# Qw11111111111/SequenceAligning

Hardware: AMD Instinct MI355X
Metric: GCUPS (affine-gap NW) at 1/2/4/8 MI355X; % of HBM roofline (higher is better)
Workload: dtype i32-exact (i16x2 packed arithmetic)

## Files before the change

sequencealigning_amd/csrc/nw_kernels.hip:

```cpp
#include <hip/hip_runtime.h>

#include <algorithm>
#include <type_traits>
#include <utility>

#include "nw_common.hpp"
#include "nw_host.hpp"
#include "saln_options.hpp"
#include "saln.h"

namespace saln {

template <int G>
__device__ __forceinline__ int32_t shr1(int32_t old, int32_t v) {
    static_assert(G == 16 || G == 64, "group must be a DPP row or the wave");
    if constexpr (G == 16)
        return __builtin_amdgcn_update_dpp(old, v, 0x111 , 0xf, 0xf, false);
    else
        return __builtin_amdgcn_update_dpp(old, v, 0x138 , 0xf, 0xf, false);
}

__device__ __forceinline__ uint32_t pack_block(uint32_t bpp, uint32_t i = blockIdx.x) {
    const uint32_t sup = 8u * bpp;
    const uint32_t r = i % sup;
// ... 893 lines not shown
            push(SALN_CIGAR_D, n);
            i -= (int32_t)n;
        }
        st = __builtin_amdgcn_readlane(nxt, L);
    }
    if (NWV > 1) {
        if (lane == 0) req[0] = -1;
        __syncthreads();
    }
    if (run_len) {
        if (lane == 0 && out) out[nops] = (run_len << 4) | run_op;
        ++nops;
    }
    if constexpr (kSpec) {
        if (lane == 0) {
            const int32_t cur = sa.pass & 1;
            rec->in_i = ei;
            rec->in_j = ej;
            rec->in_k = ek;
            rec->out_i[cur] = xi;
            rec->out_j[cur] = xj;
            rec->out_k[cur] = ev < 0 ? xk : kSpecEv + ev;
            rec->nops = nops;
            rec->am_end = am_end;
        }
        return;
    }
    if (ev != kEvOrigin) nops = 0;
    if (out && nops > 1) {
        __builtin_amdgcn_s_waitcnt(0x0F70);
        __builtin_amdgcn_fence(__ATOMIC_SEQ_CST, "workgroup");
        for (uint32_t a = (uint32_t)lane; a < nops / 2; a += 64) {
            const uint32_t x = out[a], y = out[nops - 1 - a];
            out[a] = y;
            out[nops - 1 - a] = x;
        }
    }
    if (lane == 0) {
        saln_nw_result r = make_result(hend, WalkOut{ev, nops}, am_end);
        results[p.pair_id] = r;
    }
}

__global__ __launch_bounds__(256) void nw_spec_link_kernel(
    const NwPairDesc *__restrict__ pairs, SpecArgs sa, uint32_t *__restrict__ done,
    const int32_t *__restrict__ end_h, saln_nw_result *__restrict__ results,
    uint32_t *__restrict__ strict_err) {
    __shared__ uint32_t s_n[kSpecMaxStripes], s_first[kSpecMaxStripes], s_last[kSpecMaxStripes];
    __shared__ uint8_t s_k0[kSpecMaxStripes];
    __shared__ uint32_t s_part[256];
    __shared__ int32_t t_sh, bad_sh;
    const SpecPair sp = sa.pairs[blockIdx.x];
    const int32_t S = (int32_t)sp.n_stripes, P = sa.pass & 1;
    SpecStripe *rec = sa.stripes + sp.stripe_base;
    const uint32_t *ops = sa.ops + (uint64_t)sp.stripe_base * kSpecOpsCap;
    const int32_t tid = (int32_t)threadIdx.x;
    if (tid == 0) {
        t_sh = -1;
        bad_sh = 0;
    }
    __syncthreads();
    for (int32_t s = tid; s < S; s += 256)
        if (rec[s].out_k[P] >= kSpecEv) atomicMax(&t_sh, s);
    __syncthreads();
    const int32_t t = t_sh;
    const int32_t tk = t >= 0 ? rec[t].out_k[P] : kSpecNone;
    bool bad = t < 0 || tk == kSpecNone || tk == kSpecEv + kEvDead;
    for (int32_t s = max(t, 0) + tid; !bad && s < S - 1; s += 256) {
        const SpecStripe &a = rec[s], &b = rec[s + 1];
        if (a.in_i != b.out_i[P] || a.in_j != b.out_j[P] || a.in_k != b.out_k[P]) bad_sh = 1;
    }
    __syncthreads();
    const uint32_t idx = sp.plan_idx;
    if (bad || bad_sh) {
        if (tid == 0) {
            done[idx] = 0u;
            if (strict_err) atomicOr(strict_err, 2u);
        }
        return;
    }
    for (int32_t s = tid; s < S; s += 256) {
        const uint32_t n = s >= t ? rec[s].nops : 0u;
        s_n[s] = n;
        s_first[s] = n ? ops[(uint64_t)s * kSpecOpsCap] : 0u;
        s_last[s] = n ? ops[(uint64_t)s * kSpecOpsCap + n - 1] : 0u;
        if (s < t) rec[s].k0 = (int32_t)n;
    }
    __syncthreads();
    for (int32_t s = tid; s < S; s += 256)
        s_k0[s] = (s >= t && s < S - 1 && s_n[s] && (s_first[s] & 15u) == (s_last[s + 1] & 15u))
                      ? 1u : 0u;
    __syncthreads();
    const int32_t C = (S + 255) / 256;
    const int32_t u0 = tid * C, u1 = min(S, u0 + C);
    uint32_t part = 0;
    for (int32_t u = u0; u < u1; ++u) part += s_n[S - 1 - u] - s_k0[S - 1 - u];
    s_part[tid] = part;
    __syncthreads();
    for (int32_t d = 1; d < 256; d <<= 1) {
        const uint32_t v = tid >= d ? s_part[tid - d] : 0u;
        __syncthreads();
        s_part[tid] += v;
        __syncthreads();
    }
    uint32_t g = s_part[tid] - part;
    for (int32_t u = u0; u < u1; ++u) {
        const int32_t s = S - 1 - u;
        const uint32_t n = s_n[s], k0 = s_k0[s];
        rec[s].base = (int32_t)g - (int32_t)k0;
        rec[s].k0 = (int32_t)k0;
        if (n > k0) {
            uint32_t len = s_last[s] >> 4;
            for (int32_t r = s - 1; r >= t && s_k0[r]; --r) {
                len += s_first[r] >> 4;
                if (s_n[r] != 1u) break;
            }
            rec[s].open_w = (len << 4) | (s_last[s] & 15u);
        }
        g += n - k0;
    }
    if (tid == 255) {
        const uint32_t N = s_part[255];
        const NwPairDesc p = pairs[idx];
        const int ev = tk - kSpecEv;
        results[p.pair_id] = make_result(end_h[idx], WalkOut{ev, ev == kEvOrigin ? N : 0u},
                                         rec[S - 1].am_end);
        done[idx] = 1u;
    }
}

__global__ __launch_bounds__(64) void nw_spec_copy_kernel(
    const NwPairDesc *__restrict__ pairs, SpecArgs sa, const saln_nw_result *__restrict__ results,
    uint32_t *__restrict__ cigar) {
    const uint2 b = sa.blocks[blockIdx.x];
    const SpecPair sp = sa.pairs[b.x];
    if (!sa.done[sp.plan_idx]) return;
    const NwPairDesc p = pairs[sp.plan_idx];
    const int32_t N = (int32_t)results[p.pair_id].cigar_len;
    const SpecStripe &r = sa.stripes[sp.stripe_base + b.y];
    const int32_t n = (int32_t)r.nops;
    if (N == 0 || r.k0 >= n) return;
    const uint32_t *w = sa.ops + (uint64_t)(sp.stripe_base + b.y) * kSpecOpsCap;
    uint32_t *out = cigar + p.cigar_off;
    for (int32_t k = r.k0 + (int32_t)threadIdx.x; k < n; k += 64)
        out[N - 1 - (r.base + k)] = k == n - 1 ? r.open_w : w[k];
}

template <int K>
struct MaskWords {
    uint32_t w[(K + 3) / 4];
};


constexpr uint32_t kPub = 32;
constexpr uint32_t kColEmpty = 0x80000000u;

typedef short s16x2 __attribute__((ext_vector_type(2)));
typedef unsigned short u16x2 __attribute__((ext_vector_type(2)));

__device__ __forceinline__ s16x2 as_s2(uint32_t x) { return __builtin_bit_cast(s16x2, x); }
__device__ __forceinline__ uint32_t as_u(s16x2 x) { return __builtin_bit_cast(uint32_t, x); }
__device__ __forceinline__ s16x2 spl(int32_t v) { return s16x2{(short)v, (short)v}; }
__device__ __forceinline__ uint32_t pk2(int32_t lo, int32_t hi) {
    return ((uint32_t)lo & 0xFFFFu) | ((uint32_t)hi << 16);
}
__device__ __forceinline__ s16x2 vmax(s16x2 a, s16x2 b) { return __builtin_elementwise_max(a, b); }
__device__ __forceinline__ uint32_t pkb(int32_t lo, int32_t hi) {
    return ((uint32_t)(lo + 32768) & 0xFFFFu) | ((uint32_t)(hi + 32768) << 16);
}
__device__ __forceinline__ uint32_t umax2(uint32_t a, uint32_t b) {
    return __builtin_bit_cast(uint32_t, __builtin_elementwise_max(__builtin_bit_cast(u16x2, a),
                                                                  __builtin_bit_cast(u16x2, b)));
}
__device__ __forceinline__ uint32_t umin2(uint32_t a, uint32_t b) {
    return __builtin_bit_cast(uint32_t, __builtin_elementwise_min(__builtin_bit_cast(u16x2, a),
                                                                  __builtin_bit_cast(u16x2, b)));
}
__device__ __forceinline__ uint32_t cst2(int32_t c) { return (uint32_t)c * 0x10001u; }

template <int G>
__device__ __forceinline__ uint32_t gshift(uint32_t bnd, uint32_t v, bool group_start) {
    uint32_t s;
    if constexpr (G <= 16)
        s = __builtin_amdgcn_update_dpp(bnd, v, 0x111 , 0xf, 0xf, false);
    else
        s = __builtin_amdgcn_update_dpp(bnd, v, 0x138 , 0xf, 0xf, false);
    if constexpr (G == 16 || G == 64) return s;
    return group_start ? bnd : s;
}

__device__ __forceinline__ uint32_t col_pair_signs(uint32_t hi, uint32_t lo) {
    return __builtin_amdgcn_perm(hi, lo, 0x0B0A0908u);
}

__device__ __forceinline__ uint32_t bfi(uint32_t m, uint32_t a, uint32_t b) {
    return __builtin_amdgcn_bitop3_b32(m, a, b, 0xCA);
}

template <bool kArgMBit>
__device__ __forceinline__ uint32_t merge_walk(const uint32_t (&p)[8]) {
    uint32_t r = kArgMBit ? bfi(0x01010101u, p[0], p[1]) : p[1];
    r = bfi(0x03030303u, r, p[2]);
    r = bfi(0x07070707u, r, p[4]);
    r = bfi(0x1F1F1F1Fu, r, p[6]);
    return bfi(0x7F7F7F7Fu, r, p[7]);
}
__device__ __forceinline__ uint32_t merge_full(const uint32_t (&p)[8]) {
    uint32_t r = bfi(0x01010101u, p[0], p[1]);
    r = bfi(0x03030303u, r, p[2]);
    r = bfi(0x07070707u, r, p[3]);
    r = bfi(0x0F0F0F0Fu, r, p[4]);
    r = bfi(0x1F1F1F1Fu, r, p[5]);
    r = bfi(0x3F3F3F3Fu, r, p[6]);
    return bfi(0x7F7F7F7Fu, r, p[7]);
}

template <int K>
struct PkMask {
    uint32_t w[(K + 3) / 4];
};
template <int K>
__device__ __forceinline__ uint32_t pick_col(const uint32_t (&h)[K], int k) {
    uint32_t v[K];
#pragma unroll
    for (int i = 0; i < K; ++i) v[i] = h[i];
    int n = K;
#pragma unroll
    for (int bit = 0; (1 << bit) < K; ++bit) {
        const bool b = (k >> bit) & 1;
#pragma unroll
        for (int i = 0; 2 * i < n; ++i) v[i] = 2 * i + 1 < n ? (b ? v[2 * i + 1] : v[2 * i]) : v[2 * i];
        n = (n + 1) / 2;
    }
    return v[0];
}
template <int K>
struct NibSeg {
    uint32_t w[(K + 3) / 4 / 2 + 1];
};

struct PlanSrc {
    const NwPairDesc *pairs;
    uint32_t first;
    int32_t *end_h;
    __device__ __forceinline__ NwPairDesc pair(uint32_t i) const { return pairs[first + i]; }
    __device__ __forceinline__ void end(uint32_t i, const NwPairDesc &, int32_t h) const {
        end_h[first + i] = h;
    }
};

struct AvsaSrc {
    const uint64_t *q_off, *d_off;
    const uint32_t *q_ids, *d_ids;
    uint32_t nq;
    uint32_t nq_total;
    uint64_t base;
    int2 *out;
    __device__ __forceinline__ NwPairDesc pair(uint32_t i) const {
        const uint64_t k = base + i;
        const uint32_t qi = q_ids[k % nq], di = d_ids[k / nq];
        NwPairDesc p{};
        p.q_off = q_off[qi];
        p.db_off = d_off[di];
        p.len_q = (uint32_t)(q_off[qi + 1] - p.q_off);
        p.len_db = (uint32_t)(d_off[di + 1] - p.db_off);
        p.mask_off = (uint64_t)di * nq_total + qi;
        return p;
    }
    __device__ __forceinline__ void end(uint32_t, const NwPairDesc &p, int32_t h) const {
        out[p.mask_off] = make_int2(h >> 1, (h & 1) ? SALN_REF_PANIC_BOUNDARY : SALN_OK);
    }
};

struct AvsaSrcP : AvsaSrc {
    __device__ __forceinline__ NwPairDesc pair(uint32_t i) const {
        const uint64_t k = base + i, j = k >> 1;
        const uint32_t qi = q_ids[j % nq], di = d_ids[2 * (j / nq) + (k & 1)];
        NwPairDesc p{};
        p.q_off = q_off[qi];
        p.db_off = d_off[di];
        p.len_q = (uint32_t)(q_off[qi + 1] - p.q_off);
        p.len_db = (uint32_t)(d_off[di + 1] - p.db_off);
        p.mask_off = (uint64_t)di * nq_total + qi;
        return p;
    }
};


template <int G, int K, int kCodes>
constexpr int pk_min_waves() { return kCodes == 3  && G == 8 ? 3 : 1; }
typedef _Float16 f16x2 __attribute__((ext_vector_type(2)));
__device__ __forceinline__ uint32_t hmax3(uint32_t a, uint32_t b, uint32_t c) {
    return __builtin_bit_cast(
        uint32_t, __builtin_elementwise_maximum(__builtin_bit_cast(f16x2, a),
                                                __builtin_elementwise_maximum(
                                                    __builtin_bit_cast(f16x2, b),
                                                    __builtin_bit_cast(f16x2, c))));
}

struct RowIn {
    uint32_t w;
};

template <int G, int K, int kCodes, typename Src, int KS, bool kRebase = false, bool kProf = false,
          int kTabMode = 0>
__device__ __forceinline__ int fill_pk_body(Src src, uint32_t count, const uint8_t *__restrict__ qs,
                                            const uint8_t *__restrict__ ds,
                                            uint8_t *__restrict__ mask, Scoring sc,
                                            uint32_t ld_max, bool sc_steady,
                                            uint32_t vblock = ~0u) {
    constexpr bool kTab = kTabMode == 1 || kTabMode == 4 || kTabMode == 5;
    constexpr bool kRowProf = kTabMode == 5;
    constexpr bool kFree = kTab || kTabMode == 3;
    constexpr bool kS4 = kTabMode == 4;
    constexpr int kSc = kS4 ? 4 : 2;
    auto up = [](int32_t v2) -> int32_t { return kS4 ? (v2 >> 1) * 4 + (v2 & 1) : v2; };
    static_assert(kTabMode != 3 || kProf, "kTabMode 3: query profiles");
    constexpr int32_t kBias = kFree ? kFreeBias : 32768;
    auto pkx = [](int32_t lo, int32_t hi) {
        return ((uint32_t)(lo + kBias) & 0xFFFFu) | ((uint32_t)(hi + kBias) << 16);
    };
    static_assert(!kProf || (kCodes == kCodesNone && !kRebase), "profiles: score-only, one frame");
    static_assert(!kTab || ((kCodes == kCodesNib || kCodes == kCodesNone || kCodes == kCodesFull) &&
                            !kRebase && !kProf && !(kS4 && kCodes == kCodesFull)),
                  "tables: 4-bit codes, full codes (scale 2) or score-only, one frame");
    constexpr int GPB = 256 / G;
    constexpr Geom geo{G, K};
    extern __shared__ uint32_t drow[];
    const int lane = threadIdx.x % G;
    const uint32_t gi = pack_block(blocks_per_pack(2 * GPB), vblock == ~0u ? blockIdx.x : vblock) * GPB +
                        threadIdx.x / G;
    const uint32_t ia = 2 * gi, ib = 2 * gi + 1;
    if (ia >= count) return 0;
    const bool hasB = ib < count;
    const NwPairDesc pa = src.pair(ia);
    NwPairDesc pb = pa;
    if (hasB) pb = src.pair(ib);
    const int ldA = (int)pa.len_db, ldB = hasB ? (int)pb.len_db : 0;
    const int lqA = (int)pa.len_q, lqB = hasB ? (int)pb.len_q : 0;
    const uint8_t *__restrict__ qA = qs + pa.q_off;
    const uint8_t *__restrict__ qB = qs + pb.q_off;
    const uint8_t *__restrict__ dA = ds + pa.db_off;
    const uint8_t *__restrict__ dB = ds + pb.db_off;
    const int ldM = ldA > ldB ? ldA : ldB;
    const int32_t beta = -kSc * sc.gap_extend;
    const int32_t alpha = kFree ? beta : -2 * sc.match - beta;
    const uint32_t kPen = cst2(2 * (sc.match - sc.mismatch));
    const uint32_t kOpen = cst2(kSc * sc.gap_open);
    const uint32_t kDstep = cst2(2 * sc.gap_extend + alpha);
    const int32_t drift = kFree ? 0 : 2 * sc.gap_extend + alpha;
    const uint32_t cm = (uint32_t)(kSc * sc.match + alpha + beta) & 0xFFu;
    const uint32_t cmm = (uint32_t)(kSc * sc.mismatch + alpha + beta) & 0xFFu;
    const uint32_t kBonus = cm | cmm * 0x01010100u;
    const uint32_t kProfBase = cmm * 0x01010101u, kProfStep = cm - cmm;
    const uint32_t kCmm2 = cmm * 0x00010001u;
    constexpr uint32_t kAcgt = 'A' | 'C' << 8 | 'T' << 16 | 'G' << 24;
    auto acgt = [](uint32_t c) { return c == 'A' || c == 'C' || c == 'G' || c == 'T'; };
    bool bad = false;
    const uint32_t kRebaseAdd = cst2(-drift * kRebaseSteps);
    const int32_t ctr = kRebase ? rebase_center(sc, G * K) : 0;
    const bool gstart = lane == 0;

    const int col0 = lane * K;
    uint32_t qc[K], Hp[K], Dn[K];
    const uint32_t pen1 = 2 * (sc.match - sc.mismatch);
#pragma unroll
    for (int k = 0; k < K; ++k) {
        const int j = col0 + k + 1;
        if constexpr (kProf && kFree) {
            const uint32_t qch = j <= lqA ? (uint32_t)qA[j - 1] : 0u;
            qc[k] = (qch == 'A' ? cm : cmm) | (qch == 'C' ? cm : cmm) << 8 |
                    (qch == 'T' ? cm : cmm) << 16 | (qch == 'G' ? cm : cmm) << 24;
        } else if constexpr (kProf) {
            const uint32_t qch = j <= lqA ? (uint32_t)qA[j - 1] : 0u;
            qc[k] = (qch == 'A' ? 0u : pen1) | (qch == 'C' ? 0u : pen1 << 8) |
                    (qch == 'T' ? 0u : pen1 << 16) | (qch == 'G' ? 0u : pen1 << 24);
        } else if constexpr (kTab) {
            const uint32_t ca = j <= lqA ? (uint32_t)qA[j - 1] : 'A';
            const uint32_t cb = j <= lqB ? (uint32_t)qB[j - 1] : 'A';
            bad |= !acgt(ca) || !acgt(cb);
            qc[k] = kRowProf ? (((ca >> 1) & 3u) | 0x0C00u | (((cb >> 1) & 3u) + 4u) << 16 | 0x0C000000u)
                             : (((ca >> 1) & 3u) | ((cb >> 1) & 3u) << 16);
        } else {
            const uint32_t ca = j <= lqA ? (uint32_t)qA[j - 1] << 5 : 0xE000u;
            const uint32_t cb = j <= lqB ? (uint32_t)qB[j - 1] << 5 : 0xE000u;
            if constexpr (kTabMode == 2) bad |= (j <= lqA && !acgt(ca >> 5)) || (j <= lqB && !acgt(cb >> 5));
            qc[k] = ca | (cb << 16);
        }
        const int32_t h0 = up(hs_row0(sc, (uint32_t)j)) + beta * j - ctr;
        const int32_t d1 = up(ds_row1(sc, (uint32_t)j)) + alpha + beta * j - ctr;
        Hp[k] = pkx(h0, h0);
        Dn[k] = pkx(d1, d1);
    }
    uint32_t hd = pkx(up(hs_row0(sc, (uint32_t)col0)) + beta * col0 - ctr,
                      up(hs_row0(sc, (uint32_t)col0)) + beta * col0 - ctr);
    uint32_t pubF = 0, pubH = 0;
    uint32_t *__restrict__ myrow = drow + (threadIdx.x / G) * (ld_max + 2 * G) + G;
    uint16_t *__restrict__ myrow16 = reinterpret_cast<uint16_t *>(drow) +
                                     (threadIdx.x / G) * (ld_max + 2 * G) + G;
    for (int i = lane; i < ldM; i += G) {
        const uint32_t ca = i < ldA ? (uint32_t)dA[i] : 0u;
        const uint32_t cb = i < ldB ? (uint32_t)dB[i] : 0u;
        if constexpr (kRebase) {
            if constexpr (kTabMode == 2) bad |= (i < ldA && !acgt(ca)) || (i < ldB && !acgt(cb));
            myrow16[i] = (uint16_t)(ca | (cb << 8));
        } else if constexpr (kRowProf) {
            bad |= (i < ldA && !acgt(ca)) || (i < ldB && !acgt(cb));
            myrow[i] = ((ca >> 1) & 3u) << 3 | ((cb >> 1) & 3u) << 19 | 0x60006000u;
        } else if constexpr (kTab) {
            bad |= (i < ldA && !acgt(ca)) || (i < ldB && !acgt(cb));
            myrow[i] = ((ca >> 1) & 3u) | ((cb >> 1) & 3u) << 16 | 0x0C000C00u;
        } else {
            if constexpr (kTabMode == 2) bad |= (i < ldA && !acgt(ca)) || (i < ldB && !acgt(cb));
            myrow[i] = (ca << 5) | (cb << 21);
        }
    }
    asm volatile("s_waitcnt lgkmcnt(0)" : : : "memory");
    __builtin_amdgcn_wave_barrier();
    if constexpr (kTab) {
        if (__builtin_amdgcn_ballot_w64(bad)) return 1;
    } else if constexpr (kTabMode == 2) {
        if (!__builtin_amdgcn_ballot_w64(bad)) return 2;
    }
    const int lA = (lqA - 1) / K, kA = (lqA - 1) % K;
    const int lB = hasB ? (lqB - 1) / K : -1, kB = hasB ? (lqB - 1) % K : 0;
    const int tEA = lane == lA ? ldA + lane - 1 : -1;
    const int tEB = lane == lB ? ldB + lane - 1 : -1;
    static_assert(K % KS == 0 && (KS % 2 == 0 || KS == K), "segments hold whole column pairs");
    constexpr int NS = K / KS;
    uint8_t *__restrict__ mA = mask + pa.mask_off + (uint64_t)(lane * NS) * pa.mask_bs -
                               (int64_t)lane * (int64_t)pa.mask_rs;
    uint8_t *__restrict__ mB = mask + pb.mask_off + (uint64_t)(lane * NS) * pb.mask_bs -
                               (int64_t)lane * (int64_t)pb.mask_rs;
    const uint32_t *__restrict__ rowp = myrow - lane;
    const uint16_t *__restrict__ rowp16 = myrow16 - lane;
    const int T = (int)geo.steps((uint32_t)ldM);
    constexpr bool kWalkCodes = kCodes == kCodesWalk || kCodes == kCodesNib;
    static_assert(kCodes != kCodesNib || KS == K, "4-bit codes: one segment per lane");
    const int ldAs = (kWalkCodes && col0 >= lqA) ? 0 : ldA;
    const int ldBs = (kWalkCodes && col0 >= lqB) ? 0 : ldB;
    uint32_t HpB[K];

    uint32_t sF = 0, sH = 0;
    const uint32_t kRowAdd = cst2(drift);
    auto step = [&](int t, uint32_t(&Hin)[K], uint32_t(&Hout)[K], auto steady_c, RowIn row_in)
                    __attribute__((always_inline)) {
        constexpr bool kSteady = decltype(steady_c)::value;
        constexpr bool kRun = kSteady && !kRebase;
        const int r = t - lane + 1;
        uint32_t dch;
        if constexpr (kRun)
            dch = row_in.w;
        else if constexpr (kRebase)
            dch = __builtin_amdgcn_perm(0u, (uint32_t)rowp16[t], 0x0C010C00u) << 5;
        else
            dch = rowp[t];
        uint32_t prof_lo = 0, prof_hi = 0;
        if constexpr (kRowProf) {
            prof_lo = (kProfStep << (dch & 31u)) + kProfBase;
            prof_hi = (kProfStep << ((dch >> 16) & 31u)) + kProfBase;
        }
        int32_t base = 0;
        if constexpr (kRebase) {
            base = drift * (t & -kRebaseSteps) + ctr;
            if ((t & (kRebaseSteps - 1)) == 0 && t > 0) {
#pragma unroll
                for (int k = 0; k < K; ++k) {
                    Hin[k] += kRebaseAdd;
                    Dn[k] += kRebaseAdd;
                }
                hd += kRebaseAdd;
                pubF += kRebaseAdd;
                pubH += kRebaseAdd;
            }
        }
        const int32_t rb = t + 1;
        uint32_t gF, gH;
        if constexpr (kRun) {
            gF = sF;
            gH = sH;
            sF += kRowAdd;
            sH += kRowAdd;
        } else {
            const int32_t bF = up(is_col1(sc, (uint32_t)rb)) + alpha * rb + beta - base;
            const int32_t bH = up(hs_col0(sc, (uint32_t)rb)) + alpha * rb - base;
            gF = pkx(bF, bF);
            gH = pkx(bH, bH);
        }
        const uint32_t inF = gshift<G>(gF, pubF, gstart);
        const uint32_t inH = gshift<G>(gH, pubH, gstart);
        if (kSteady || (r >= 1 && r <= ldM)) {
            uint32_t F = inF;
            PkMask<KS> wa[NS], wb[NS];
            uint32_t cw[(K + 1) / 2];
            uint32_t prv[8];
            uint32_t nw[(K + 3) / 4], nlo = 0, nprv[4];
            const uint32_t endsel = (t == tEA ? 0x0000FFFFu : 0u) | (t == tEB ? 0xFFFF0000u : 0u);
            const uint32_t psel = kProf ? (((dch >> 6) & 0x00030003u) | 0x0C000C00u) : 0u;
            auto columns = [&](auto with_argm) __attribute__((always_inline)) {
            constexpr bool kM = decltype(with_argm)::value;
            uint32_t diag = hd;
#pragma unroll
            for (int k = 0; k < K; ++k) {
                const uint32_t hdk = diag;
                diag = Hin[k];
                const uint32_t pen = kProf     ? __builtin_amdgcn_perm(0u, qc[k], psel)
                                     : kRowProf ? __builtin_amdgcn_perm(prof_hi, prof_lo, qc[k])
                                     : kTab     ? __builtin_amdgcn_perm(0u, kBonus, qc[k] ^ dch)
                                                : umin2(qc[k] ^ dch, kPen);
                const uint32_t M = kFree ? hdk + pen : hdk - pen;
                const uint32_t I = F, D = Dn[k];
                const uint32_t H = kFree ? hmax3(M, I, D) : umax2(M, umax2(I, D));
                const uint32_t tO = M + kOpen;
                if constexpr (kCodes == kCodesNib) {
                    uint32_t s4[4];
                    if constexpr (kS4) {
                        const uint32_t Hm = H - 0x00020002u;
                        const uint32_t tO2 = M + (kOpen + 0x00020002u);
                        s4[0] = Hm - I;
                        s4[1] = Hm - D;
                        s4[2] = tO2 - I;
                        s4[3] = tO2 - D;
                        if constexpr (kM) s4[3] = bfi(endsel, M - Hm, s4[3]);
                    } else {
                    const uint32_t Hc = H & 0xFFFEFFFEu;
                    const uint32_t tOr = tO | 0x00010001u;
                    auto psub = [](uint32_t a, uint32_t b) { return as_u(as_s2(a) - as_s2(b)); };
                    s4[0] = psub(I, Hc);
                    s4[1] = psub(D, Hc);
                    s4[2] = psub(tOr, I);
                    s4[3] = psub(tOr, D);
                    if constexpr (kM) s4[3] = bfi(endsel, psub(M, Hc), s4[3]);
                    }
                    if (k % 2 == 0 && k < K - 1) {
#pragma unroll
                        for (int u = 0; u < 4; ++u) nprv[u] = s4[u];
                    } else {
                        uint32_t pw[4];
#pragma unroll
                        for (int u = 0; u < 4; ++u)
                            pw[u] = k % 2 ? col_pair_signs(s4[u], nprv[u])
                                          : col_pair_signs(kS4 && u < 2 ? 0x80008000u : 0u, s4[u]);
                        const int cp = k / 2, g = cp / 2;
                        auto bfi01 = [](uint32_t m, uint32_t a, uint32_t b) {
                            return kS4 ? __builtin_amdgcn_bitop3_b32(m, a, b, 0x35) : bfi(m, a, b);
                        };
                        if (cp % 2 == 0) {
                            uint32_t lo = bfi01(0x01010101u, pw[0], pw[1]);
                            lo = bfi(0x03030303u, lo, pw[2]);
                            lo = bfi(0x07070707u, lo, pw[3]);
                            if (cp == (K - 1) / 2) nw[g] = lo;
                            else nlo = lo;
                        } else {
                            uint32_t x = bfi01(0x10101010u, pw[0], pw[1]);
                            x = bfi(0x30303030u, x, pw[2]);
                            x = bfi(0x70707070u, x, pw[3]);
                            nw[g] = bfi(0x0F0F0F0Fu, nlo, x);
                        }
                    }
                } else if constexpr (kCodes != kCodesNone) {
                const uint32_t Hc = H & 0xFFFEFFFEu;
                const uint32_t tOr = tO | 0x00010001u;
                auto psub = [](uint32_t a, uint32_t b) { return as_u(as_s2(a) - as_s2(b)); };
                uint32_t sg[8];
                sg[0] = kM ? psub(M, Hc) : 0u;
                sg[1] = psub(I, Hc);
                sg[2] = psub(D, Hc);
                sg[4] = psub(tOr, I);
                sg[6] = psub(tOr, D);
                sg[7] = kFree ? psub(kCmm2, pen) : pen - 0x00010001u;
                if constexpr (kCodes == kCodesFull) {
                    const uint32_t tOc = tO & 0xFFFEFFFEu;
                    sg[3] = psub(I, tOc);
                    sg[5] = psub(D, tOc);
                } else {
                    sg[3] = sg[5] = 0u;
                }
                if (k % 2 == 0 && k < K - 1) {
#pragma unroll
                    for (int t = 0; t < 8; ++t) prv[t] = sg[t];
                } else {
                    uint32_t pw[8];
#pragma unroll
                    for (int t = 0; t < 8; ++t)
                        pw[t] = k % 2 ? col_pair_signs(sg[t], prv[t]) : col_pair_signs(0u, sg[t]);
                    cw[k / 2] = kCodes == kCodesFull ? merge_full(pw) : merge_walk<kM>(pw);
                }
                }
                F = umax2(tO, I);
                Dn[k] = kFree ? umax2(tO, D) : umax2(tO, D) + kDstep;
                Hout[k] = H;
            }
            };
            if constexpr (kWalkCodes && kSteady) {
                columns(std::false_type{});
            } else if constexpr (kWalkCodes) {
                const bool endcell = t == tEA || t == tEB;
                if (__builtin_amdgcn_ballot_w64(endcell))
                    columns(std::true_type{});
                else
                    columns(std::false_type{});
            } else {
                columns(std::true_type{});
            }
            hd = inH;
            pubF = F;
            pubH = Hout[K - 1];
            if constexpr (kCodes == kCodesNib) {
                constexpr int NG = (K + 3) / 4, ND = NG / 2 + 1;
                const uint32_t rot = kRowProf ? __builtin_amdgcn_perm(0u, kAcgt, dch >> 3)
                                     : kTab   ? __builtin_amdgcn_perm(0u, kAcgt, dch)
                                              : __builtin_amdgcn_alignbit(dch, dch, 5);
                NibSeg<K> na, nb;
#pragma unroll
                for (int d = 0; d < NG / 2; ++d) {
                    na.w[d] = __builtin_amdgcn_perm(nw[2 * d + 1], nw[2 * d], 0x06040200u);
                    nb.w[d] = __builtin_amdgcn_perm(nw[2 * d + 1], nw[2 * d], 0x07050301u);
                }
                if constexpr (NG % 2) {
                    na.w[ND - 1] = __builtin_amdgcn_perm(rot, nw[NG - 1], 0x0C040200u);
                    nb.w[ND - 1] = __builtin_amdgcn_perm(rot, nw[NG - 1], 0x0C060301u);
                } else {
                    na.w[ND - 1] = rot & 0xFFu;
                    nb.w[ND - 1] = __builtin_amdgcn_ubfe(rot, 16, 8);
                }
                if (kSteady ? ldAs != 0 : r <= ldAs) *reinterpret_cast<NibSeg<K> *>(mA) = na;
                if (kSteady ? ldBs != 0 : r <= ldBs) *reinterpret_cast<NibSeg<K> *>(mB) = nb;
            } else if constexpr (kCodes != kCodesNone) {
#pragma unroll
                for (int sg = 0; sg < NS; ++sg) {
#pragma unroll
                    for (int w = 0; w < (KS + 3) / 4; ++w) {
                        const uint32_t lo = cw[sg * KS / 2 + 2 * w];
                        const uint32_t hi = 2 * w + 1 < (KS + 1) / 2 ? cw[sg * KS / 2 + 2 * w + 1] : 0u;
                        wa[sg].w[w] = __builtin_amdgcn_perm(hi, lo, 0x06040200u);
                        wb[sg].w[w] = __builtin_amdgcn_perm(hi, lo, 0x07050301u);
                    }
                }
                if (kSteady ? ldAs != 0 : r <= ldAs) {
#pragma unroll
                    for (int sg = 0; sg < NS; ++sg)
                        *reinterpret_cast<PkMask<KS> *>(mA + (uint64_t)sg * pa.mask_bs) = wa[sg];
                }
                if (kSteady ? ldBs != 0 : r <= ldBs) {
#pragma unroll
                    for (int sg = 0; sg < NS; ++sg)
                        *reinterpret_cast<PkMask<KS> *>(mB + (uint64_t)sg * pb.mask_bs) = wb[sg];
                }
            }
            auto down = [](int32_t v) -> int32_t { return kS4 ? (v >> 2) * 2 + (v & 1) : v; };
            if (!kSteady && t == tEA) {
                const int32_t e = (int32_t)(pick_col<K>(Hout, kA) & 0xFFFFu) - kBias;
                src.end(ia, pa, down(e + base - alpha * ldA - beta * lqA));
            }
            if (!kSteady && t == tEB) {
                const int32_t e = (int32_t)(pick_col<K>(Hout, kB) >> 16) - kBias;
                src.end(ib, pb, down(e + base - alpha * ldB - beta * lqB));
            }
        } else if (&Hout != &Hin) {
#pragma unroll
            for (int k = 0; k < K; ++k) Hout[k] = Hin[k];
        }
        mA += pa.mask_rs;
        mB += pb.mask_rs;
    };
    const std::false_type G0;
    const std::true_type S1;
    const int ldm = ldA < (hasB ? ldB : ldA) ? ldA : (hasB ? ldB : ldA);
    const int tS0 = min((G + 1) & ~1, T & ~1);
    const int tS1 = sc_steady ? max(tS0, tS0 + ((ldm - 1 - tS0) & ~1) * (ldm - 1 > tS0 ? 1 : 0)) : tS0;
    int t = 0;
    const RowIn z{};
    auto rowin = [&](int tt) __attribute__((always_inline)) {
        if constexpr (kRebase) return z;
        else return RowIn{rowp[tt]};
    };
    for (; t < tS0; t += 2) {
        step(t, Hp, HpB, G0, z);
        step(t + 1, HpB, Hp, G0, z);
    }
    if (tS1 > tS0) {
        if constexpr (!kRebase) {
            const int32_t rb = tS0 + 1;
            const int32_t bF = up(is_col1(sc, (uint32_t)rb)) + alpha * rb + beta;
            const int32_t bH = up(hs_col0(sc, (uint32_t)rb)) + alpha * rb;
            sF = pkx(bF, bF);
            sH = pkx(bH, bH);
        }
        RowIn d0 = rowin(t);
        for (; t < tS1; t += 2) {
            const RowIn d1 = rowin(t + 1);
            step(t, Hp, HpB, S1, d0);
            d0 = rowin(t + 2);
            step(t + 1, HpB, Hp, S1, d1);
        }
    }
    for (; t + 1 < T; t += 2) {
        step(t, Hp, HpB, G0, z);
        step(t + 1, HpB, Hp, G0, z);
    }
    if (t < T) step(t, Hp, HpB, G0, z);
    return 0;
}

template <int G, int K, int kCodes, typename Src, int KS, bool kRebase = false>
__global__ __launch_bounds__(256, (pk_min_waves<G, K, kCodes>())) void nw_fill_pk_kernel(
    Src src, uint32_t count, const uint8_t *__restrict__ qs, const uint8_t *__restrict__ ds,
    uint8_t *__restrict__ mask, Scoring sc, uint32_t ld_max, bool sc_steady) {
    fill_pk_body<G, K, kCodes, Src, KS, kRebase>(src, count, qs, ds, mask, sc, ld_max, sc_steady);
}

template <int G, int K, typename Src, int kScale = 2, int kCodes = kCodesNib>
__global__ __launch_bounds__(256, (pk_min_waves<G, K, kCodes>())) void nw_fill_pk_tab_kernel(
    Src src, uint32_t count, const uint8_t *__restrict__ qs, const uint8_t *__restrict__ ds,
    uint8_t *__restrict__ mask, Scoring sc, uint32_t ld_max, uint32_t *__restrict__ bail,
    uint32_t epoch) {
    __builtin_amdgcn_s_setprio(2);
    const int st = fill_pk_body<G, K, kCodes, Src, K, false, false,
                                kScale == 4 ? 4 : kScale == 3 ? 5 : 1>(src, count, qs, ds, mask,
                                                                       sc, ld_max, true);
    if (__builtin_amdgcn_ballot_w64(st == 1) && (threadIdx.x & 63u) == 0) *bail = epoch;
}
template <int G, int K, typename Src, bool kRebaseGeneric, int kCodes = kCodesNib>
__global__ __launch_bounds__(256, (pk_min_waves<G, K, kCodes>())) void nw_fill_pk_tabfb_kernel(
    Src src, uint32_t count, const uint8_t *__restrict__ qs, const uint8_t *__restrict__ ds,
    uint8_t *__restrict__ mask, Scoring sc, uint32_t ld_max, const uint32_t *__restrict__ bail,
    uint32_t epoch, uint32_t vblocks) {
    if (__builtin_amdgcn_readfirstlane(*bail) != epoch) return;
    for (uint32_t vb = blockIdx.x; vb < vblocks; vb += gridDim.x)
        fill_pk_body<G, K, kCodes, Src, K, kRebaseGeneric, false, 2>(src, count, qs, ds, mask, sc,
                                                                      ld_max, true, vb);
}

template <int G, int K, bool kRebaseGeneric>
__global__ __launch_bounds__(256, (pk_min_waves<G, K, kCodesNone>())) void nw_fill_avsa_tab_kernel(
    AvsaSrc src, uint32_t count, const uint8_t *__restrict__ qs, const uint8_t *__restrict__ ds,
    Scoring sc, uint32_t ld_max, bool sc_steady, const uint32_t *__restrict__ generic) {
    if (__builtin_amdgcn_readfirstlane(*generic))
        fill_pk_body<G, K, kCodesNone, AvsaSrc, K, kRebaseGeneric, false, 0>(
            src, count, qs, ds, nullptr, sc, ld_max, sc_steady);
    else
        fill_pk_body<G, K, kCodesNone, AvsaSrc, K, false, false, 1>(src, count, qs, ds, nullptr, sc,
                                                                    ld_max, sc_steady);
}

template <int G, int K, bool kFree>
__global__ __launch_bounds__(256) void nw_fill_avsa_prof_kernel(
    AvsaSrcP src, uint32_t count, const uint8_t *__restrict__ qs, const uint8_t *__restrict__ ds,
    Scoring sc, uint32_t ld_max, bool sc_steady, const uint32_t *__restrict__ generic) {
    if (__builtin_amdgcn_readfirstlane(*generic))
        fill_pk_body<G, K, kCodesNone, AvsaSrcP, K, false, false>(src, count, qs, ds, nullptr, sc,
                                                                  ld_max, sc_steady);
    else
        fill_pk_body<G, K, kCodesNone, AvsaSrcP, K, false, true, kFree ? 3 : 0>(
            src, count, qs, ds, nullptr, sc, ld_max, sc_steady);
}

__global__ __launch_bounds__(256) void nw_acgt_check_kernel(const uint8_t *__restrict__ seq,
                                                            uint64_t n, uint32_t *__restrict__ flag) {
    bool bad = false;
    for (uint64_t i = (uint64_t)blockIdx.x * 256 + threadIdx.x; i < n; i += (uint64_t)gridDim.x * 256) {
        const uint8_t c = seq[i];
        bad |= c != 'A' && c != 'C' && c != 'G' && c != 'T';
    }
    if (__builtin_amdgcn_ballot_w64(bad) && (threadIdx.x & 63u) == 0) atomicOr(flag, 1u);
}

template <int kCodes, bool kArgM, bool kEq = true>
__device__ __forceinline__ uint32_t stripe_code_word(const uint32_t (&s)[8][4]) {
    uint32_t w[8];
#pragma unroll
    for (int t = 0; t < 8; ++t) {
        if ((t == 0 && kCodes != kCodesFull && !kArgM) || (t == 7 && kCodes != kCodesFull && !kEq) ||
            ((t == 3 || t == 5) && kCodes != kCodesFull)) {
            w[t] = 0u;
            continue;
        }
        w[t] = __builtin_amdgcn_perm(s[t][1], s[t][0], 0x0C0C0B09u) |
               __builtin_amdgcn_perm(s[t][3], s[t][2], 0x0B090C0Cu);
    }
    if constexpr (kCodes == kCodesFull) return merge_full(w);
    if constexpr (!kEq) {
        uint32_t r = kArgM ? bfi(0x01010101u, w[0], w[1]) : w[1];
        r = bfi(0x03030303u, r, w[2]);
        r = bfi(0x07070707u, r, w[4]);
        return bfi(0x1F1F1F1Fu, r, w[6]);
    }
    return merge_walk<kArgM>(w);
}
template <int kCodes>
__device__ __forceinline__ uint32_t stripe_code_word(const uint32_t (&s)[8][4]) {
    return stripe_code_word<kCodes, true>(s);
}

constexpr int32_t kNegInf = INT32_MIN;
constexpr uint32_t kRowsOff = 0;
constexpr uint32_t kRowsGrp = 8;

template <class Fill>
__device__ __forceinline__ int32_t wave_prefix_max(int32_t v, Fill &&fill) {
    v = max(v, __builtin_amdgcn_update_dpp(kNegInf, v, 0x111 , 0xf, 0xf, false));
    fill();
    v = max(v, __builtin_amdgcn_update_dpp(kNegInf, v, 0x112 , 0xf, 0xf, false));
    v = max(v, __builtin_amdgcn_update_dpp(kNegInf, v, 0x114 , 0xf, 0xf, false));
    v = max(v, __builtin_amdgcn_update_dpp(kNegInf, v, 0x118 , 0xf, 0xf, false));
    v = max(v, __builtin_amdgcn_update_dpp(kNegInf, v, 0x142 , 0xa, 0xf, false));
    v = max(v, __builtin_amdgcn_update_dpp(kNegInf, v, 0x143 , 0xc, 0xf, false));
    return v;
}

constexpr int kPlaceShared = 0, kPlaceLone = 1, kPlaceXcd = 2;
template <int K, int kCodes, bool kMinPen, int kPlace>
__global__ __launch_bounds__(64) void nw_fill_rows_kernel(
    const NwPairDesc *__restrict__ pairs, const uint2 *__restrict__ work,
    const uint8_t *__restrict__ qs, const uint8_t *__restrict__ ds, uint8_t *__restrict__ mask,
    int2 *__restrict__ scratch, uint32_t *__restrict__ err, int32_t *__restrict__ end_h,
    Scoring sc, uint32_t n_waves, uint32_t xcd_run, uint32_t epoch) {
    static_assert(K == 1 || K == 2, "4 cells per code word (K = 4, 256-column stripes: slower, round 2)");
    constexpr int S = 4 / K;
    constexpr int W = 64 * K;
    if constexpr (kPlace != kPlaceShared) asm volatile("" : : : "a255");
    const int lane = (int)(threadIdx.x & 63u);
    const uint32_t v = __builtin_amdgcn_readfirstlane(
        kPlace == kPlaceXcd ? (blockIdx.x & 7u) * xcd_run + (blockIdx.x >> 3) : blockIdx.x);
    if (v >= n_waves) return;
    bool plain_pub = false;
    if constexpr (kPlace == kPlaceXcd) {
        uint32_t *const slots = err + 2;
        const uint32_t xcc = __builtin_amdgcn_s_getreg((31 << 11) | 20) & 15u;
        const uint32_t me = (epoch << 4) | xcc;
        if (lane == 0) asm volatile("global_store_dword %0, %1, off sc1" : : "v"(slots + v), "v"(me) : "memory");
        if ((v + 1) % xcd_run != 0 && v + 1 < n_waves) {
            uint32_t got = 0;
            for (uint32_t k = 0; k < 4096u; ++k) {
                asm volatile("global_load_dword %0, %1, off sc1\n\ts_waitcnt vmcnt(0)"
                             : "=v"(got) : "v"(slots + v + 1) : "memory");
                if ((got >> 4) == ((epoch << 4) >> 4)) break;
                __builtin_amdgcn_s_sleep(2);
            }
            plain_pub = __builtin_amdgcn_readfirstlane(got) == me;
        }
    }
    const uint2 wk = work[v / S];
    const NwPairDesc p = pairs[wk.x];
    const uint32_t g = wk.y * S + v % S;
    const uint32_t lq = p.len_q, ld = p.len_db;
    const uint32_t c0 = g * W;
    if (c0 >= lq) return;
    const uint32_t nst = (lq + W - 1) / W;
    const int2 *__restrict__ scr_in = g > 0 ? scratch + p.scratch_off + (uint64_t)(g - 1) * scratch_col(ld) : nullptr;
    int2 *__restrict__ scr_out = scratch + p.scratch_off + (uint64_t)g * scratch_col(ld);
    (void)nst;
    const int32_t beta = -4 * sc.gap_extend;
    const int32_t alpha = -4 * sc.match - beta;
    const int32_t pen_max = 4 * (sc.match - sc.mismatch);
    const int32_t kOpen = 4 * sc.gap_open;
    const int32_t kDstep = 4 * sc.gap_extend + alpha;
    constexpr int32_t kTieOr = kCodes == kCodesFull ? 3 : 1;
    const uint32_t col0 = c0 + (uint32_t)lane * K;
    uint32_t qc[K];
    int32_t Hp[K], Dn[K];
#pragma unroll
    for (int k = 0; k < K; ++k) {
        const uint32_t j = col0 + k + 1;
        qc[k] = j <= lq ? (uint32_t)qs[p.q_off + j - 1] << 8 : 0xFFFFFF00u;
        Hp[k] = hs4_row0(sc, j) + beta * (int32_t)j;
        Dn[k] = ds4_row1(sc, j) + alpha + beta * (int32_t)j;
    }
    int32_t hb_prev = hs4_row0(sc, c0) + beta * (int32_t)c0;
    int32_t cH_v = hb_prev, cH_prev_v = hb_prev;
    uint8_t *mrow = mask + p.mask_off + (uint64_t)(c0 / 256) * p.mask_cs + (col0 % 256);
    typedef const __attribute__((address_space(4))) uint32_t cu32;
    const uint8_t *d = ds + p.db_off;
    cu32 *dw = (cu32 *)((uintptr_t)d & ~(uintptr_t)3);
    const uint32_t doff = 8u * (uint32_t)((uintptr_t)d & 3);
    const uint32_t last_dw = ((uint32_t)ld - 1 + (uint32_t)((uintptr_t)d & 3)) >> 2;
    uint32_t dnidx = min(1u, last_dw);
    uint32_t dcur = dw[0], dnxt = dw[dnidx];

    bool failed = false;
    const int2 *pub_base = scr_out;
    uint32_t pub_voff = 0;
    const uint32_t jend = lq - 1;
    const bool end_lane = jend / W == g && (uint32_t)lane == (jend % W) / K;
    const uint32_t k_end = jend % K;
    __builtin_amdgcn_s_waitcnt(0x0F70);
    uint32_t sg[8][4];
    constexpr bool kCodesHere = kCodes != kCodesNone;
    auto row = [&](uint32_t r, uint32_t dch, int32_t bH, int32_t bI, auto u_c, auto q_c,
                   auto m_c, auto &&fill, auto vb_c, auto plain_c) __attribute__((always_inline)) {
        constexpr int u = decltype(u_c)::value;
        constexpr int q = decltype(q_c)::value;
        constexpr bool kM = decltype(m_c)::value;
        const int32_t hm = (kCodes == kCodesFull || (kM && r == ld)) ? ~3 : ~1;
        int32_t M[K], tO[K], P[K], Dv[K];
        uint32_t s6[K];
        int32_t hbv;
        if constexpr (decltype(vb_c)::value) {
            if constexpr (q == 0)
                hbv = __builtin_amdgcn_update_dpp(0, cH_prev_v, 0x107 , 0xf, 0xf, true);
            else if constexpr (q == 1)
                hbv = cH_v;
            else
                hbv = __builtin_amdgcn_update_dpp(0, cH_v, 0x100 + (q - 1) , 0xf, 0xf, true);
        } else {
            hbv = hb_prev;
        }
        int32_t diag = __builtin_amdgcn_update_dpp(hbv, Hp[K - 1], 0x138 , 0xf, 0xf, false);
        uint32_t x[K];
#pragma unroll
        for (int k = 0; k < K; ++k) {
            x[k] = qc[k] ^ dch;
            const int32_t pen = kMinPen ? (int32_t)min(x[k], (uint32_t)pen_max) : (x[k] ? pen_max : 0);
            M[k] = (k == 0 ? diag : Hp[k - 1]) - pen;
            tO[k] = M[k] + kOpen;
            P[k] = k == 0 ? tO[0] : max(P[k - 1], tO[k]);
            Dv[k] = Dn[k];
            s6[k] = (uint32_t)((tO[k] | kTieOr) - Dv[k]);
            Dn[k] = max(tO[k], Dv[k]) + kDstep;
        }
        const int32_t S_incl = wave_prefix_max(P[K - 1], fill);
        const int32_t Ein = max(__builtin_amdgcn_update_dpp(kNegInf, S_incl, 0x138, 0xf, 0xf, false), bI);
#pragma unroll
        for (int k = 0; k < K; ++k) {
            const int32_t I = k == 0 ? Ein : max(Ein, P[k - 1]);
            const int32_t D = Dv[k];
            const int32_t H = max(M[k], max(I, D));
            if constexpr (kCodesHere) {
                const int32_t Hc = H & hm;
                const int32_t tOr = tO[k] | kTieOr;
                const int e = u * K + k;
                sg[0][e] = (kCodes == kCodesFull || kM) ? (uint32_t)(M[k] - Hc) : 0u;
                sg[1][e] = (uint32_t)(I - Hc);
                sg[2][e] = (uint32_t)(D - Hc);
                sg[4][e] = (uint32_t)(tOr - I);
                sg[6][e] = s6[k];
                sg[7][e] = kCodes == kCodesFull ? x[k] - 1u : 0u;
                if constexpr (kCodes == kCodesFull) {
                    const int32_t tOc = tO[k] & ~3;
                    sg[3][e] = (uint32_t)(I - tOc);
                    sg[5][e] = (uint32_t)(D - tOc);
                } else {
                    sg[3][e] = sg[5][e] = 0u;
                }
            }
            Hp[k] = H;
        }
        hb_prev = bH;
        {
            const int32_t iv = max(S_incl, bI);
            const uint64_t val = (uint64_t)(uint32_t)Hp[K - 1] | ((uint64_t)(uint32_t)iv << 32);
            const uint32_t vo = pub_voff;
            const int2 *pb = pub_base;
            if constexpr (decltype(plain_c)::value)
                asm volatile("global_store_dwordx2 %0, %1, %2 offset:%3"
                             : : "v"(vo), "v"(val), "s"(pb), "i"(8 * q) : "memory");
            else
                asm volatile("global_store_dwordx2 %0, %1, %2 offset:%3 sc1"
                             : : "v"(vo), "v"(val), "s"(pb), "i"(8 * q) : "memory");
        }
    };
    auto put = [&](uint32_t r0, uint32_t n, auto m_c) __attribute__((always_inline)) {
        if constexpr (kCodesHere) {
            const uint32_t wv = stripe_code_word<kCodes, decltype(m_c)::value, false>(sg);
            uint8_t *a = mrow + (uint64_t)(r0 - 1) * 256;
            if constexpr (K == 2) {
                *reinterpret_cast<uint16_t *>(a) = (uint16_t)wv;
                if (n > 1) *reinterpret_cast<uint16_t *>(a + 256) = (uint16_t)(wv >> 16);
            } else {
                a[0] = (uint8_t)wv;
                if (n > 1) a[256] = (uint8_t)(wv >> 8);
                if (n > 2) a[512] = (uint8_t)(wv >> 16);
                if (n > 3) a[768] = (uint8_t)(wv >> 24);
            }
        }
    };
    auto nofill = []() __attribute__((always_inline)) {};
    const std::integral_constant<int, 0> u0;
    const std::integral_constant<int, 1> u1;
    const std::integral_constant<int, 2> u2;
    const std::integral_constant<int, 3> u3;
    auto rows = [&](auto F, auto PL) __attribute__((always_inline)) {
        constexpr bool kFirst = decltype(F)::value;
        const std::integral_constant<bool, !kFirst> VB;
        constexpr uint32_t kG = kRowsGrp;
        uint64_t nv = 0;
        auto fetch = [&](uint32_t r0) __attribute__((always_inline)) {
            if (!kFirst && lane < (int)kG && r0 + (uint32_t)lane <= ld)
                asm volatile("global_load_dwordx2 %0, %1, off sc1"
                             : "=v"(nv) : "v"(scr_in + r0 + kRowsOff + lane) : "memory");
        };
        fetch(1);
        if constexpr (!kFirst) asm volatile("s_waitcnt vmcnt(0)" : "+v"(nv) : : "memory");
        int32_t bh[kG], bi[kG];
        auto group = [&](uint32_t r, auto next_c) __attribute__((always_inline)) {
            constexpr bool kNext = decltype(next_c)::value;
            pub_base = scr_out + r;
            pub_voff = lane == 63 ? 0u : (ld + 1u - r) * 8u;
            if constexpr (kFirst) {
// ... 1142 lines not shown
```

Measured before the change: 2713.

## Load query and database sequences as aligned words with batched prefetch

Replaces the byte-wise loads of query and database characters in the fill kernel prologue with aligned 32-bit word loads realigned by alignbyte. Database chars are issued in several batches ahead of the LDS stores to overlap latency. ACGT validation is vectorized with a perm lookup, and byte unpacking uses perm/ubfe. Also drops wave priority before the tail loop in table mode. This cuts global load instruction count and prologue latency, at the cost of more registers and clamped-edge loads that must stay within the sequence bounds.

```diff
diff --git a/sequencealigning_amd/csrc/nw_kernels.hip b/sequencealigning_amd/csrc/nw_kernels.hip
--- a/sequencealigning_amd/csrc/nw_kernels.hip
+++ b/sequencealigning_amd/csrc/nw_kernels.hip
@@ -1219,6 +1219,33 @@
     uint32_t w;
 };
 
+template <int N>
+__device__ __forceinline__ void seq_words_issue(const uint8_t *__restrict__ s, uint32_t n, int32_t o,
+                                                uint32_t (&raw)[N + 1]) {
+    const int32_t al = (int32_t)((uintptr_t)s & 3u);
+    const int32_t first = ((al + o) & ~3) - al, last = ((al + (int32_t)n - 1) & ~3) - al;
+#pragma unroll
+    for (int i = 0; i <= N; ++i) {
+        const int32_t a = first + 4 * i;
+        raw[i] = *reinterpret_cast<const uint32_t *>(s + (a < last ? a : last));
+    }
+}
+template <int N>
+__device__ __forceinline__ void seq_words(const uint8_t *s, int32_t o, const uint32_t (&raw)[N + 1],
+                                          uint32_t (&w)[N]) {
+    const uint32_t sh = (uint32_t)((uintptr_t)s + (uint32_t)o) & 3u;
+#pragma unroll
+    for (int i = 0; i < N; ++i) w[i] = __builtin_amdgcn_alignbyte(raw[i + 1], raw[i], sh);
+}
+__device__ __forceinline__ uint32_t seq_pad(uint32_t w, int32_t nv, uint32_t pad) {
+    const uint32_t keep = nv >= 4 ? ~0u : nv <= 0 ? 0u : (1u << (8 * (nv & 3))) - 1u;
+    return bfi(keep, w, pad);
+}
+__device__ __forceinline__ uint32_t not_acgt4(uint32_t w) {
+    constexpr uint32_t kAcgt = 'A' | 'C' << 8 | 'T' << 16 | 'G' << 24;
+    return __builtin_amdgcn_perm(0u, kAcgt, (w >> 1) & 0x03030303u) ^ w;
+}
+
 template <int G, int K, int kCodes, typename Src, int KS, bool kRebase = false, bool kProf = false,
           int kTabMode = 0>
 __device__ __forceinline__ int fill_pk_body(Src src, uint32_t count, const uint8_t *__restrict__ qs,
@@ -1251,8 +1278,7 @@
     if (ia >= count) return 0;
     const bool hasB = ib < count;
     const NwPairDesc pa = src.pair(ia);
-    NwPairDesc pb = pa;
-    if (hasB) pb = src.pair(ib);
+    const NwPairDesc pb = src.pair(hasB ? ib : ia);
     const int ldA = (int)pa.len_db, ldB = hasB ? (int)pb.len_db : 0;
     const int lqA = (int)pa.len_q, lqB = hasB ? (int)pb.len_q : 0;
     const uint8_t *__restrict__ qA = qs + pa.q_off;
@@ -1272,7 +1298,6 @@
     const uint32_t kProfBase = cmm * 0x01010101u, kProfStep = cm - cmm;
     const uint32_t kCmm2 = cmm * 0x00010001u;
     constexpr uint32_t kAcgt = 'A' | 'C' << 8 | 'T' << 16 | 'G' << 24;
-    auto acgt = [](uint32_t c) { return c == 'A' || c == 'C' || c == 'G' || c == 'T'; };
     bool bad = false;
     const uint32_t kRebaseAdd = cst2(-drift * kRebaseSteps);
     const int32_t ctr = kRebase ? rebase_center(sc, G * K) : 0;
@@ -1281,29 +1306,90 @@
     const int col0 = lane * K;
     uint32_t qc[K], Hp[K], Dn[K];
     const uint32_t pen1 = 2 * (sc.match - sc.mismatch);
+    uint32_t *__restrict__ myrow = drow + (threadIdx.x / G) * (ld_max + 2 * G) + G;
+    uint16_t *__restrict__ myrow16 = reinterpret_cast<uint16_t *>(drow) +
+                                     (threadIdx.x / G) * (ld_max + 2 * G) + G;
+    constexpr int NQ = (K + 3) / 4;
+    constexpr int kDbB = G >= 32 ? 2 : G >= 16 ? 3 : 5;
+    constexpr uint32_t kA4 = 0x41414141u;
+    uint32_t qrA[NQ + 1], qrB[NQ + 1], dr[kDbB][2][2];
+    seq_words_issue<NQ>(qA, pa.len_q, col0, qrA);
+    if constexpr (!kProf) seq_words_issue<NQ>(qB, pb.len_q, col0, qrB);
+    auto db_issue = [&](int m0) __attribute__((always_inline)) {
+#pragma unroll
+        for (int u = 0; u < kDbB; ++u) {
+            const int32_t o = 4 * (m0 + lane + G * u);
+            seq_words_issue<1>(dA, pa.len_db, o, dr[u][0]);
+            seq_words_issue<1>(dB, pb.len_db, o, dr[u][1]);
+        }
+    };
+    auto db_store = [&](int m0) __attribute__((always_inline)) {
+#pragma unroll
+        for (int u = 0; u < kDbB; ++u) {
+            const int i0 = 4 * (m0 + lane + G * u);
+            if (i0 >= ldM) continue;
+            uint32_t wa[1], wb[1];
+            seq_words<1>(dA, i0, dr[u][0], wa);
+            seq_words<1>(dB, i0, dr[u][1], wb);
+            if constexpr (kTab || kTabMode == 2)
+                bad |= (not_acgt4(seq_pad(wa[0], ldA - i0, kA4)) |
+                        not_acgt4(seq_pad(wb[0], ldB - i0, kA4))) != 0;
+            uint32_t a = seq_pad(wa[0], ldA - i0, 0u), b = seq_pad(wb[0], ldB - i0, 0u);
+            if constexpr (kTab) {
+                a = (a >> 1) & 0x03030303u;
+                b = (b >> 1) & 0x03030303u;
+            }
+#pragma unroll
+            for (int c = 0; c < 4; ++c) {
+                if constexpr (kRebase) {
+                    myrow16[i0 + c] = (uint16_t)__builtin_amdgcn_perm(b, a, 0x0C0C0400u + 0x0101u * c);
+                } else {
+                    const uint32_t x = __builtin_amdgcn_perm(b, a, 0x0C040C00u + 0x00010001u * c);
+                    myrow[i0 + c] = kRowProf ? (x << 3 | 0x60006000u) : kTab ? (x | 0x0C000C00u) : x << 5;
+                }
+            }
+        }
+    };
+    db_issue(0);
+    {
+        uint32_t wA[NQ], wB[NQ];
+        seq_words<NQ>(qA, col0, qrA, wA);
+        if constexpr (!kProf) seq_words<NQ>(qB, col0, qrB, wB);
+#pragma unroll
+        for (int i = 0; i < NQ; ++i) {
+            const int32_t nvA = lqA - col0 - 4 * i, nvB = lqB - col0 - 4 * i;
+            if constexpr (kTab || kTabMode == 2)
+                bad |= (not_acgt4(seq_pad(wA[i], nvA, kA4)) | not_acgt4(seq_pad(wB[i], nvB, kA4))) != 0;
+            wA[i] = seq_pad(wA[i], nvA, 0u);
+            if constexpr (!kProf) wB[i] = seq_pad(wB[i], nvB, 0u);
+            if constexpr (kTab) {
+                wA[i] = (wA[i] >> 1) & 0x03030303u;
+                wB[i] = ((wB[i] >> 1) & 0x03030303u) + (kRowProf ? 0x04040404u : 0u);
+            }
+        }
+#pragma unroll
+        for (int k = 0; k < K; ++k) {
+            const int j = col0 + k + 1;
+            const uint32_t qch = __builtin_amdgcn_ubfe(wA[k / 4], 8 * (k % 4), 8);
+            if constexpr (kProf && kFree) {
+                qc[k] = (qch == 'A' ? cm : cmm) | (qch == 'C' ? cm : cmm) << 8 |
+                        (qch == 'T' ? cm : cmm) << 16 | (qch == 'G' ? cm : cmm) << 24;
+            } else if constexpr (kProf) {
+                qc[k] = (qch == 'A' ? 0u : pen1) | (qch == 'C' ? 0u : pen1 << 8) |
+                        (qch == 'T' ? 0u : pen1 << 16) | (qch == 'G' ? 0u : pen1 << 24);
+            } else if constexpr (kTab) {
+                const uint32_t x = __builtin_amdgcn_perm(wB[k / 4], wA[k / 4],
+                                                         0x0C040C00u + 0x00010001u * (k % 4));
+                qc[k] = kRowProf ? (x | 0x0C000C00u) : x;
+            } else {
+                const uint32_t cb = __builtin_amdgcn_ubfe(wB[k / 4], 8 * (k % 4), 8);
+                qc[k] = (j <= lqA ? qch << 5 : 0xE000u) | (j <= lqB ? cb << 5 : 0xE000u) << 16;
+            }
+        }
+    }
 #pragma unroll
     for (int k = 0; k < K; ++k) {
         const int j = col0 + k + 1;
-        if constexpr (kProf && kFree) {
-            const uint32_t qch = j <= lqA ? (uint32_t)qA[j - 1] : 0u;
-            qc[k] = (qch == 'A' ? cm : cmm) | (qch == 'C' ? cm : cmm) << 8 |
-                    (qch == 'T' ? cm : cmm) << 16 | (qch == 'G' ? cm : cmm) << 24;
-        } else if constexpr (kProf) {
-            const uint32_t qch = j <= lqA ? (uint32_t)qA[j - 1] : 0u;
-            qc[k] = (qch == 'A' ? 0u : pen1) | (qch == 'C' ? 0u : pen1 << 8) |
-                    (qch == 'T' ? 0u : pen1 << 16) | (qch == 'G' ? 0u : pen1 << 24);
-        } else if constexpr (kTab) {
-            const uint32_t ca = j <= lqA ? (uint32_t)qA[j - 1] : 'A';
-            const uint32_t cb = j <= lqB ? (uint32_t)qB[j - 1] : 'A';
-            bad |= !acgt(ca) || !acgt(cb);
-            qc[k] = kRowProf ? (((ca >> 1) & 3u) | 0x0C00u | (((cb >> 1) & 3u) + 4u) << 16 | 0x0C000000u)
-                             : (((ca >> 1) & 3u) | ((cb >> 1) & 3u) << 16);
-        } else {
-            const uint32_t ca = j <= lqA ? (uint32_t)qA[j - 1] << 5 : 0xE000u;
-            const uint32_t cb = j <= lqB ? (uint32_t)qB[j - 1] << 5 : 0xE000u;
-            if constexpr (kTabMode == 2) bad |= (j <= lqA && !acgt(ca >> 5)) || (j <= lqB && !acgt(cb >> 5));
-            qc[k] = ca | (cb << 16);
-        }
         const int32_t h0 = up(hs_row0(sc, (uint32_t)j)) + beta * j - ctr;
         const int32_t d1 = up(ds_row1(sc, (uint32_t)j)) + alpha + beta * j - ctr;
         Hp[k] = pkx(h0, h0);
@@ -1312,25 +1398,10 @@
     uint32_t hd = pkx(up(hs_row0(sc, (uint32_t)col0)) + beta * col0 - ctr,
                       up(hs_row0(sc, (uint32_t)col0)) + beta * col0 - ctr);
     uint32_t pubF = 0, pubH = 0;
-    uint32_t *__restrict__ myrow = drow + (threadIdx.x / G) * (ld_max + 2 * G) + G;
-    uint16_t *__restrict__ myrow16 = reinterpret_cast<uint16_t *>(drow) +
-                                     (threadIdx.x / G) * (ld_max + 2 * G) + G;
-    for (int i = lane; i < ldM; i += G) {
-        const uint32_t ca = i < ldA ? (uint32_t)dA[i] : 0u;
-        const uint32_t cb = i < ldB ? (uint32_t)dB[i] : 0u;
-        if constexpr (kRebase) {
-            if constexpr (kTabMode == 2) bad |= (i < ldA && !acgt(ca)) || (i < ldB && !acgt(cb));
-            myrow16[i] = (uint16_t)(ca | (cb << 8));
-        } else if constexpr (kRowProf) {
-            bad |= (i < ldA && !acgt(ca)) || (i < ldB && !acgt(cb));
-            myrow[i] = ((ca >> 1) & 3u) << 3 | ((cb >> 1) & 3u) << 19 | 0x60006000u;
-        } else if constexpr (kTab) {
-            bad |= (i < ldA && !acgt(ca)) || (i < ldB && !acgt(cb));
-            myrow[i] = ((ca >> 1) & 3u) | ((cb >> 1) & 3u) << 16 | 0x0C000C00u;
-        } else {
-            if constexpr (kTabMode == 2) bad |= (i < ldA && !acgt(ca)) || (i < ldB && !acgt(cb));
-            myrow[i] = (ca << 5) | (cb << 21);
-        }
+    db_store(0);
+    for (int m0 = G * kDbB; 4 * m0 < ldM; m0 += G * kDbB) {
+        db_issue(m0);
+        db_store(m0);
     }
     asm volatile("s_waitcnt lgkmcnt(0)" : : : "memory");
     __builtin_amdgcn_wave_barrier();
@@ -1612,6 +1683,7 @@
             step(t + 1, HpB, Hp, S1, d1);
         }
     }
+    if constexpr (kTab) __builtin_amdgcn_s_setprio(0);
     for (; t + 1 < T; t += 2) {
         step(t, Hp, HpB, G0, z);
         step(t + 1, HpB, Hp, G0, z);
```

Measured after the change: 2761, median of 6. 1.8% higher.
